# iamgroot42/A-LINK

Measured on AMD Instinct MI355X. Metric: 112x112 face embeddings/sec (IR-ResNet-100 ArcFace, 512-d, L2-normalised), higher is better.
Workload: dtype bf16

## Files before the change

a-link_amd/csrc/alink_common.h:

```cpp
#pragma once
#include <hip/hip_runtime.h>
#include <stdint.h>
#include <stddef.h>
#include <string>

#include "../../include/alink_hip.h"
#include "conv_kernel.h"

namespace alink {

void set_error(const char* fmt, ...);
int  hip_fail(hipError_t e, const char* what, const char* file, int line);

#define ALINK_HIP(call)                                                          \
    do {                                                                         \
        hipError_t e__ = (call);                                                 \
        if (e__ != hipSuccess) return ::alink::hip_fail(e__, #call, __FILE__, __LINE__); \
    } while (0)

#define ALINK_REQUIRE(cond, code, ...)          \
    do {                                        \
        if (!(cond)) {                          \
            ::alink::set_error(__VA_ARGS__);    \
            return (code);                      \
// ... 19 lines not shown
        if (dev < 0 || hipGetDevice(&prev) != hipSuccess || prev == dev) return;
        switched = hipSetDevice(dev) == hipSuccess;
    }
    ~DeviceGuard() {
        if (switched) (void)hipSetDevice(prev);
    }
    DeviceGuard(const DeviceGuard&) = delete;
    DeviceGuard& operator=(const DeviceGuard&) = delete;
};

typedef __attribute__((ext_vector_type(8))) __bf16   bf16x8;
typedef __attribute__((ext_vector_type(8))) _Float16 f16x8;
typedef __attribute__((ext_vector_type(4))) float    f32x4;
typedef __attribute__((ext_vector_type(16))) float   f32x16;

struct ConvParams {
    const void*  in;
    const void*  wgt;
    const float* bias;
    const float* alpha;
    const void*  resid;
    const void*  dact;
    void*        out;
    const void*  zero;
    const void*  in2;
    int Cin2;
    int in2_compact;
    int N, H, W, Cin, Cout, Ho, Wo, stride, ksz, pad, M;
    int border_cls;
    int splitk;
    int ksteps_per_split;
    int post_relu;
    int fine;
    int stagger;
    int ablate;
    float acc_scale;
    float bias_scale;
    float res_scale;
    int nprod;
    void* stamps;
};

hipError_t launch_conv_igemm(int dtype, const ConvParams& p, hipStream_t stream);
double     conv_flops(const ConvParams& p);

struct StemParams {
    const void*  in;
    const void*  wgt;
    const float* bias;
    const float* alpha;
    void*        out;
    int N, H, W, C0, layout;
    float sub[3], mul;
    int flip;
    float acc_scale, bias_scale;
};
hipError_t launch_stem(int dtype, const StemParams& p, hipStream_t stream);

struct FcFinishParams {
    const float* slabs;
    const float* bias;
    float*       out;
    float*       norms;
    int S, M, E;
    float scale;
    int*  nonfinite;
// ... 77 lines not shown
```

a-link_amd/csrc/backbone.hip:

```cpp
#include "alink_common.h"
#include "net_host.h"

#include <algorithm>
#include <cmath>
#include <cstdarg>
#include <cstdio>
#include <cstring>
#include <map>
#include <string>
#include <vector>

namespace alink {

static thread_local char g_err[1024] = "";
void set_error(const char* fmt, ...) {
    va_list ap;
    va_start(ap, fmt);
    vsnprintf(g_err, sizeof(g_err), fmt, ap);
    va_end(ap);
}
int hip_fail(hipError_t e, const char* what, const char* file, int line) {
    set_error("HIP error %d (%s) in `%s` at %s:%d", (int)e, hipGetErrorString(e), what, file, line);
    return ALINK_EHIP;
}
// ... 551 lines not shown
        worst = std::max(worst, sum);
    }
    return worst;
}

static int plan_split(const alink_backbone* bb, const ConvLayer& L, int N) {
    if (!bb->split_small || N > SPLIT_MAX_N || L.Cin2) return 1;
    const long long M = (long long)N * L.Hout * L.Wout;
    const int ncc = L.Cin / 64;
    const ConvKernelTraits t = traits(L.kernel);
    long long nwg;
    int units, kpu;
    if (t.split == SplitUnit::Chunk) {
        nwg = linear_grid(M, L.Cout, t.channel_block);
        units = ncc; kpu = 9;
    } else if (t.split == SplitUnit::KStep) {
        const bool wide = (L.Cout % 128) == 0;
        nwg = wide ? ((M + 127) / 128) * (L.Cout / 128) : ((M + 255) / 256) * (L.Cout / 64);
        units = L.ksz * L.ksz * ncc; kpu = 1;
    } else {
        return 1;
    }
    if (nwg > 64) return 1;
    int best = 1;
    for (int S = 2; S <= 8; ++S)
        if (units % S == 0 && units / S * kpu >= 4 && nwg * S <= 512 && (size_t)S * M * L.Cout * 4 <= SPLIT_SLAB_BYTES) best = S;
    return best;
}

int g_sibling_aware = 1;
extern "C" void alink_debug_set_sibling_aware(int on) { g_sibling_aware = on != 0; }
int g_fine_max = 384;
extern "C" void alink_debug_set_fine_max(int n) { g_fine_max = n; }
static int fine_form(ConvKernel k, long long M, int Cout, int siblings = 1) {
    if (!traits(k).fine) return 0;
    const int sib = (g_sibling_aware && k != ConvKernel::Linear7) ? siblings : 1;
    return linear_grid(M, Cout, 128) * sib <= g_fine_max ? 1 : 0;
}
int g_ablate = 0;
int g_stop_after = 0;
extern "C" void alink_debug_set_stop_after(int n) { g_stop_after = n; }
int g_stagger = 0;
int g_shard_stagger = 0;
extern "C" void alink_debug_set_shard_stagger(int on) { g_shard_stagger = on; }

int g_fuse_unit = 1;
constexpr int FUSE_UNIT_MIN_N = 64;
extern "C" void alink_debug_set_fuse_unit(int mode) { g_fuse_unit = mode; }
extern "C" void alink_debug_set_stagger(int n) { g_stagger = n < 0 ? 0 : n; }
void* g_stamps = nullptr;
int g_prof_reps = 4;
extern "C" void alink_debug_set_profile_reps(int n) { g_prof_reps = n < 1 ? 1 : n; }
extern "C" void alink_debug_set_ablate(int a) { g_ablate = a; }
extern "C" void alink_debug_set_stamps(void* p) { g_stamps = p; }

static const ConvLayer* fusable_unit(const alink_backbone* bb, const ConvLayer& L, int N, int S, bool cache) {
    if (!g_fuse_unit || (g_fuse_unit == 1 && N < FUSE_UNIT_MIN_N) || cache || S != 1 || g_ablate || g_stamps) return nullptr;
    const int dt = bb->cfg.dtype;
    if (dt != ALINK_DT_BF16 && dt != ALINK_DT_F16) return nullptr;
    const size_t i = (size_t)(&L - bb->convs.data());
    if (L.role != 1 || i + 1 >= bb->convs.size()) return nullptr;
    const ConvLayer& L2 = bb->convs[i + 1];
    if (L2.role != 3 || L2.unit != L.unit || L2.Cin2 || L2.in_buf != L.out_buf || L2.resid_buf != L.in_buf) return nullptr;
    if (L.kernel != ConvKernel::Linear56 || L2.kernel != ConvKernel::Linear56 || L.stride != 1 || L2.stride != 1) return nullptr;
    if (L.Cin != 64 || L.Cout != 64 || L2.Cin != 64 || L2.Cout != 64 || L.Hin != 56 || L.Win != 56) return nullptr;
    if (plan_split(bb, L2, N) != 1) return nullptr;
    return &L2;
}

constexpr int FUSE_UNIT1_MIN_N = 64;
// ... 63 lines not shown
        bexp[0] = bb->stem_e_out;
    } else {
        for (int r = 0; r < reps; ++r) ALINK_HIP(launch_stem(cfg.dtype, sp, stream));
    }
    if (!front) {
        note(2.0 * N * cfg.height * cfg.width * 64.0 * 27.0, 0);
        if ((rc = mark())) return rc;
    }

    int last_out = 0, n_done = 0;
    bool front_marked = false;
    bool skip_conv2 = false;
    for (ConvLayer& L : bb->convs) {
        if (skip_conv2) { skip_conv2 = false; continue; }
        if (g_stop_after && n_done++ >= g_stop_after) return ALINK_OK;
        if (front_done && !front_marked && L.stage >= 1) {
            ALINK_HIP(hipEventRecord(front_done, stream));
            front_marked = true;
        }
        ConvParams p{};
        p.in = buf(L.in_buf); p.wgt = L.d_w; p.bias = L.d_bias; p.alpha = L.d_alpha;
        p.resid = L.resid_buf >= 0 ? buf(L.resid_buf) : nullptr;
        p.out = buf(L.out_buf); p.zero = bb->d_zero;
        if (cache) {
            if (L.role == 1) p.out = base + cache->toff[L.unit];
            if (L.role == 3) p.in = base + cache->toff[L.unit];
        }
        conv_geometry(p, N, L.Hin, L.Win, L.Cin, L.Cout, L.ksz, L.stride, L.pad, L.Cin2, x2);
        p.border_cls = L.border_cls ? 1 : 0;
        if (L.Cin2) { p.in2 = buf(L.in2_buf); p.Cin2 = L.Cin2; p.in2_compact = (front && &L == &bb->convs[1]) ? 1 : 0; }
        p.ablate = g_ablate;
        p.stagger = g_stagger;
        p.nprod = (x2 && !calib) ? bb->products : 0;
        p.fine = fine_form(L.kernel, p.M, L.Cout, bb->siblings);
        int S = plan_split(bb, L, N);
        if (S > 1) {
            ConvParams probe = p;
            probe.splitk = 1;
            if (traits(L.kernel).split == SplitUnit::Chunk ? conv3x3_lat_applies(cfg.dtype, probe) : conv_gemm_lat_applies(cfg.dtype, probe)) S = 1;
        }
        if (x2) {
            rc = bb->cal.settle(calib, &L.e_out, p.out, (size_t)p.M * L.Cout * 2, stream, [&](int e) -> int {
                p.acc_scale = std::ldexp(1.f, e - bexp[L.in_buf] - L.e_w);
                p.bias_scale = std::ldexp(1.f, e);
                p.res_scale = L.resid_buf >= 0 ? std::ldexp(1.f, e - bexp[L.resid_buf]) : 1.f;
                for (int r = 0; r < reps; ++r) ALINK_HIP(launch_conv_maybe_split(L.kernel, cfg.dtype, p, S, buf(6), stream));
                return ALINK_OK;
            });
            if (rc) return rc;
            bexp[L.out_buf] = L.e_out;
        } else if (front && &L == &bb->convs[0] && fusable_unit1(bb, front, N, cache != nullptr)) {
            const ConvLayer& L2 = bb->convs[1];
            ConvParams p2 = p;
            p2.in = buf(L2.in_buf); p2.wgt = L2.d_w; p2.bias = L2.d_bias; p2.alpha = L2.d_alpha; p2.resid = nullptr;
            p2.out = buf(L2.out_buf); p2.border_cls = L2.border_cls ? 1 : 0;
            conv_geometry(p2, N, L2.Hin, L2.Win, L2.Cin, L2.Cout, L2.ksz, L2.stride, L2.pad, L2.Cin2);
            p2.in2 = buf(L2.in2_buf); p2.Cin2 = L2.Cin2; p2.in2_compact = 1;
            ALINK_REQUIRE(unit1_c64_applies(cfg.dtype, p, sp, p2), ALINK_EINVAL, "fused unit %s: launch forms do not apply", L.name.c_str());
            for (int r = 0; r < reps; ++r) ALINK_HIP(launch_unit1_c64(cfg.dtype, p, sp, p2, bb->front_slopes_le_1, stream));
            note(conv_flops(p) + 2.0 * N * cfg.height * cfg.width * 64.0 * 27.0, 1);
            if ((rc = mark())) return rc;
            if (prof && nl < cap) split_pairs.push_back(nl - 1);
            note(conv_flops(p2), 1);
            if ((rc = mark())) return rc;
            last_out = L2.out_buf;
            skip_conv2 = true;
            continue;
// ... 358 lines not shown

static int conv_nhwc_impl(int dtype, const void* dev_in, const void* dev_w, const float* dev_bias,
                          const float* dev_alpha, const void* dev_resid, void* dev_out, int N, int H, int W, int Cin,
                          int Cout, int ksz, int stride, int pad, int border_cls, int fine, const ConvExtras& x, void* stream) {
    ALINK_REQUIRE(dev_in && dev_w && dev_bias && dev_out, ALINK_EINVAL, "NULL argument");
    DeviceGuard dg(device_of_pointer(dev_in));
    ALINK_REQUIRE(Cin % 64 == 0 && Cout % 64 == 0, ALINK_EINVAL, "Cin/Cout must be multiples of 64");
    ALINK_REQUIRE(ksz == 1 || ksz == 3, ALINK_EINVAL, "ksz must be 1 or 3");
    ALINK_REQUIRE(!border_cls || (ksz == 3 && stride == 1 && pad == 1), ALINK_EINVAL,
                  "border classes need a 3x3 stride-1 pad-1 convolution");
    ALINK_REQUIRE(dtype == ALINK_DT_BF16 || dtype == ALINK_DT_F16, ALINK_EINVAL, "dtype must be bf16 or f16");
    int rc = init_kernels();
    if (rc) return rc;
    const ConvKernel kernel = x.route ? direct_variant_tiles(ksz, stride, pad, H, W, Cin, Cout)
                                      : direct_variant(ksz, stride, pad, H, W, Cin, Cout);
    if ((rc = check_extras(kernel, dtype, ksz, Cin, dev_alpha, dev_resid, x))) return rc;
    hipStream_t st = (hipStream_t)stream;
    const int K = ksz * ksz * Cin, Cin2 = x.in2 ? x.Cin2 : 0;
    std::vector<uint16_t> h((size_t)Cout * K), h2((size_t)Cout * Cin2);
    ALINK_HIP(hipStreamSynchronize(st));
    ALINK_HIP(hipMemcpy(h.data(), dev_w, h.size() * 2, hipMemcpyDeviceToHost));
    if (Cin2) ALINK_HIP(hipMemcpy(h2.data(), x.w2, h2.size() * 2, hipMemcpyDeviceToHost));
    const std::vector<uint16_t> hp =
        pack_conv_weights(weight_layout(kernel, ksz, Cin, false, Cin2), dtype, Round16::Direct, Cout,
                          [&](int co, int tap, int ci) { return (double)widen16(dtype, h[(size_t)co * K + (size_t)tap * Cin + ci]); },
                          [&](int co, int ci) { return (double)widen16(dtype, h2[(size_t)co * Cin2 + ci]); }).w;
    ConvParams p{};
    p.in = dev_in; p.bias = dev_bias; p.alpha = dev_alpha; p.resid = dev_resid; p.dact = x.dact; p.out = dev_out;
    conv_geometry(p, N, H, W, Cin, Cout, ksz, stride, pad, Cin2);
    p.border_cls = border_cls;
    p.post_relu = x.post_relu;
    if (Cin2) { p.in2 = x.in2; p.Cin2 = Cin2; p.in2_compact = x.in2_compact ? 1 : 0; }
    p.ablate = g_ablate; p.stamps = g_stamps;
    if (traits(kernel).fine) p.fine = fine < 0 ? fine_form(kernel, p.M, Cout) : (fine ? 1 : 0);
    DeviceAllocs mem;
    void *d_wp = nullptr, *d_zero = nullptr, *d_slabs = nullptr;
    if ((rc = mem.upload(hp, &d_wp)) || (rc = mem.zeros(4096, &d_zero))) return rc;
    if (x.splitk > 1 && (rc = mem.alloc((size_t)x.splitk * p.M * Cout * 4, &d_slabs))) return rc;
    p.wgt = d_wp; p.zero = d_zero;
    hipError_t e = launch_conv_reported(kernel, dtype, p, x.splitk, (float*)d_slabs, x, st);
    hipError_t e2 = hipStreamSynchronize(st);
    if (e != hipSuccess) return hip_fail(e, "launch_conv", __FILE__, __LINE__);
    if (e2 != hipSuccess) return hip_fail(e2, "hipStreamSynchronize", __FILE__, __LINE__);
    return ALINK_OK;
}

int alink_conv_nhwc(int dtype, const void* dev_in, const void* dev_w, const float* dev_bias,
                    const float* dev_alpha, const void* dev_resid, void* dev_out, int N, int H, int W, int Cin,
                    int Cout, int ksz, int stride, int pad, int border_cls, int fine, void* stream) {
    return conv_nhwc_impl(dtype, dev_in, dev_w, dev_bias, dev_alpha, dev_resid, dev_out, N, H, W, Cin, Cout, ksz, stride, pad,
                          border_cls, fine, ConvExtras{}, stream);
}

int alink_conv_nhwc_ex(int dtype, const void* dev_in, const void* dev_w, const float* dev_bias,
                       const float* dev_alpha, const void* dev_resid, void* dev_out, int N, int H, int W, int Cin,
                       int Cout, int ksz, int stride, int pad, int border_cls, int fine, int route, const void* dev_dact,
                       int post_relu, const void* dev_in2, const void* dev_w2, int Cin2, int in2_compact, int splitk,
                       int* kernel_out, int* form_out, void* stream) {
    ConvExtras x;
    x.route = route ? 1 : 0; x.dact = dev_dact; x.post_relu = post_relu ? 1 : 0;
    x.in2 = dev_in2; x.w2 = dev_w2; x.Cin2 = Cin2; x.in2_compact = in2_compact; x.splitk = splitk;
    x.kernel = kernel_out; x.form = form_out;
    if (kernel_out) *kernel_out = -1;
    if (form_out) *form_out = -1;
    return conv_nhwc_impl(dtype, dev_in, dev_w, dev_bias, dev_alpha, dev_resid, dev_out, N, H, W, Cin, Cout, ksz, stride, pad,
                          border_cls, fine, x, stream);
}
// ... 22 lines not shown
        ALINK_HIP(hipMemcpy(h.data(), dev, h.size() * 4, hipMemcpyDeviceToHost));
        q.assign(rows * C * 2, 0);
        for (size_t m = 0; m < rows; ++m)
            for (int c = 0; c < C; ++c) {
                const size_t at = m * 2 * C + (size_t)(c >> 6) * 128 + (c & 63);
                split16(std::ldexp((double)h[m * C + c], e), &q[at], &q[at + 64]);
            }
        return ALINK_OK;
    };
    std::vector<uint16_t> qin, qres, qw;
    if ((rc = pack_act(dev_in, Min, Cin, e_in, qin))) return rc;
    if (dev_resid && (rc = pack_act(dev_resid, M, Cout, e_res, qres))) return rc;
    {
        std::vector<float> h((size_t)Cout * K);
        ALINK_HIP(hipMemcpy(h.data(), dev_w, h.size() * 4, hipMemcpyDeviceToHost));
        qw = pack_conv_weights(weight_layout(kernel, ksz, Cin, true), ALINK_DT_F16X2, Round16::Direct, Cout,
                               [&](int co, int tap, int ci) { return (double)h[(size_t)co * K + (size_t)tap * Cin + ci]; },
                               [](int, int) { return 0.0; }, &e_w).w;
    }
    DeviceAllocs mem;
    void *d_in = nullptr, *d_res = nullptr, *d_w = nullptr, *d_out = nullptr, *d_zero = nullptr, *d_slabs = nullptr;
    if ((rc = mem.upload(qin, &d_in)) || (rc = mem.upload(qw, &d_w)) || (rc = mem.alloc(M * Cout * 4, &d_out)) ||
        (rc = mem.zeros(4096, &d_zero))) return rc;
    if (x.splitk > 1 && (rc = mem.alloc((size_t)x.splitk * M * Cout * 4, &d_slabs))) return rc;
    if (dev_resid && (rc = mem.upload(qres, &d_res))) return rc;
    ConvParams p{};
    p.in = d_in; p.wgt = d_w; p.bias = dev_bias; p.alpha = dev_alpha; p.resid = d_res; p.out = d_out;
    p.zero = d_zero; p.border_cls = border_cls;
    conv_geometry(p, N, H, W, Cin, Cout, ksz, stride, pad, 0, true);
    p.post_relu = x.post_relu; p.nprod = x.nprod;
    p.acc_scale = std::ldexp(1.f, e_out - e_in - e_w);
    p.bias_scale = std::ldexp(1.f, e_out);
    p.res_scale = std::ldexp(1.f, e_out - e_res);
    if (traits(kernel).fine) p.fine = fine < 0 ? fine_form(kernel, p.M, Cout) : (fine ? 1 : 0);
    ALINK_HIP(launch_conv_reported(kernel, ALINK_DT_F16X2, p, x.splitk, (float*)d_slabs, x, st));
    ALINK_HIP(hipStreamSynchronize(st));
    std::vector<uint16_t> qo(M * Cout * 2);
    ALINK_HIP(hipMemcpy(qo.data(), d_out, qo.size() * 2, hipMemcpyDeviceToHost));
    std::vector<float> ho(M * Cout);
    for (size_t m = 0; m < M; ++m)
        for (int c = 0; c < Cout; ++c) {
            const size_t at = m * 2 * Cout + (size_t)(c >> 6) * 128 + (c & 63);
            _Float16 hh, ll;
            memcpy(&hh, &qo[at], 2);
            memcpy(&ll, &qo[at + 64], 2);
            ho[m * Cout + c] = (float)std::ldexp((double)hh + (double)ll, -e_out);
        }
    ALINK_HIP(hipMemcpy(dev_out, ho.data(), ho.size() * 4, hipMemcpyHostToDevice));
    return ALINK_OK;
}

int alink_conv_nhwc_x2(const float* dev_in, const float* dev_w, const float* dev_bias, const float* dev_alpha,
                       const float* dev_resid, float* dev_out, int N, int H, int W, int Cin, int Cout, int ksz, int stride,
                       int pad, int border_cls, int fine, int e_in, int e_w, int e_out, int e_res, void* stream) {
    return conv_nhwc_x2_impl(dev_in, dev_w, dev_bias, dev_alpha, dev_resid, dev_out, N, H, W, Cin, Cout, ksz, stride, pad, border_cls,
                             fine, e_in, e_w, e_out, e_res, ConvExtras{}, stream);
}

int alink_conv_nhwc_x2_ex(const float* dev_in, const float* dev_w, const float* dev_bias, const float* dev_alpha,
                          const float* dev_resid, float* dev_out, int N, int H, int W, int Cin, int Cout, int ksz, int stride,
                          int pad, int border_cls, int fine, int e_in, int e_w, int e_out, int e_res, int nprod, int splitk,
                          int post_relu, int* kernel_out, int* form_out, void* stream) {
    ConvExtras x;
    x.nprod = nprod; x.splitk = splitk; x.post_relu = post_relu ? 1 : 0; x.kernel = kernel_out; x.form = form_out;
    if (kernel_out) *kernel_out = -1;
    if (form_out) *form_out = -1;
    return conv_nhwc_x2_impl(dev_in, dev_w, dev_bias, dev_alpha, dev_resid, dev_out, N, H, W, Cin, Cout, ksz, stride, pad, border_cls,
// ... 5 lines not shown
```

a-link_amd/csrc/conv3x3_linear.hip:

```cpp
#include "conv_device.h"

namespace alink {
namespace {

template <int A>
struct IC { static constexpr int a = A; };

constexpr int GPX = 224;
constexpr int TPW = 7;
constexpr int NT = 256;

template <int W, int TCW>
struct Lin {
    static constexpr int BN = 2 * TCW * 16;
    static constexpr int XPIX = GPX + 2 * W + 2;
    static constexpr int XSLOTS = (XPIX * 8 + NT - 1) / NT;
    static constexpr int XBYTES = XSLOTS * NT * 16;
    static constexpr int WOFF = XBYTES;
    static constexpr int WBYTES = BN * 128;
    static constexpr size_t lds_bytes() { return (size_t)WOFF + 2 * WBYTES + 10 * BN * 4; }
    static_assert(GPX % W == 0, "a workgroup covers whole rows");
};

template <typename T, int W, int TCW, int EPI, bool SP, int NP = 3>
__global__ __launch_bounds__(NT, 2) void conv3x3_linear_kernel(const ConvParams p) {
    typedef typename Vec8<T>::type vec8;
    typedef Lin<W, TCW> G;
    constexpr int BN = G::BN, XSLOTS = G::XSLOTS, WBYTES = G::WBYTES, WSLOTS = BN * 8 / NT;
    extern __shared__ __attribute__((aligned(16))) char smem[];

    const int tid = threadIdx.x, lane = tid & 63;
    const int wave = __builtin_amdgcn_readfirstlane(tid >> 6);
    const int wpx = wave >> 1, wco = wave & 1;
    if (p.stagger > 0) {
        __shared__ int s_late;
        if (tid == 0) s_late = (int)(__builtin_amdgcn_s_getreg(6148) & 1u);
        __syncthreads();
        if (s_late)
            for (int i = 0; i < p.stagger; ++i) __builtin_amdgcn_s_sleep(16);
    }
    const int q = lane >> 4, lr = lane & 15;
    const int H = p.H, Cin = p.Cin;
    unsigned long long* const stamps = (unsigned long long*)p.stamps;
    unsigned long long refill_cycles = 0;
    if (stamps && tid == 0) stamps[(size_t)blockIdx.x * 8 + 0] = __builtin_amdgcn_s_memtime();
    constexpr int NPH = SP ? NP : 1;
    const int CinP = SP ? 2 * Cin : Cin;
    const int ncc_all = Cin >> 6;
    const int ncc = ncc_all / p.splitk, cc_first = (int)blockIdx.y * ncc;
    const int nk = ncc * 9 * NPH;
    const int K = 9 * CinP;
    const long long totpix = (long long)p.N * H * W;

    const int ntn = p.Cout / BN;
    const int lid = xcd_remap(blockIdx.x, gridDim.x);
    const int tile_n = lid % ntn, grp = lid / ntn;
    const int n0 = tile_n * BN;
    const long long gp0 = (long long)grp * GPX;

    const T* __restrict__ gin = (const T*)p.in;
    const T* __restrict__ gw = (const T*)p.wgt;
    const T* __restrict__ gz = (const T*)p.zero;

    const int xpos0 = tid >> 3;
    const int xc16 = (tid & 7) ^ ((tid >> 4) & 7);
    const long long xgp0 = gp0 - W - 1 + xpos0;
    auto stage_x = [&](int cc, int part = 0) {
        long long x0 = xgp0;
        if (SP) asm volatile("" : "+v"(x0));
#pragma unroll
        for (int i = 0; i < XSLOTS; ++i) {
            const long long gp = x0 + 32 * i;
            const bool ok = xpos0 + 32 * i < G::XPIX && gp >= 0 && gp < totpix;
            const T* src = ok ? gin + ((size_t)gp * CinP + (SP ? 2 * cc + part : cc) * 64 + xc16 * 8) : gz + (lane & 7) * 8;
            dma16(src, smem + (NT * i + wave * 64) * 16);
        }
    };
    const unsigned woff0 = (unsigned)((tid >> 3) * K + (((tid & 7) ^ ((tid >> 4) & 7)) * 8));
    const T* wstep = gw + (size_t)n0 * K + (size_t)cc_first * (SP ? 18 : 9) * 64;
    int wr = 0;
    auto stage_w = [&](int bufoff) {
#pragma unroll
        for (int i = 0; i < WSLOTS; ++i)
            dma16(wstep + (woff0 + (unsigned)(32 * i * K)), smem + G::WOFF + bufoff + (NT * i + wave * 64) * 16);
        if (SP && NP == 1) {
            wstep += wr == 8 ? 10 * 64 : 64;
            wr = wr == 8 ? 0 : wr + 1;
        } else if (SP) {
            wstep += wr == 17 ? -17 * 64 : (wr == 26 ? 10 * 64 : 64);
            wr = wr == 26 ? 0 : wr + 1;
        } else {
            wstep += 64;
        }
    };

    stage_x(cc_first);
    stage_w(0);

    const int dl = delta(lr);
    const int xbase = wpx * (TPW * 2048);
    unsigned border = 0;
#pragma unroll
    for (int u = 0; u < TPW; ++u) {
        const int pl = 16 * (wpx * TPW + u) + dl;
        const int col = pl % W;
        const int y = (int)(((unsigned)grp * (unsigned)(GPX / W) + (unsigned)(pl / W)) % (unsigned)W);
        border |= ((y == 0 ? 1u : 0u) | (y == H - 1 ? 2u : 0u) | (col == 0 ? 4u : 0u) | (col == W - 1 ? 8u : 0u)) << (4 * u);
    }
    int wl[2];
    {
        const int rowb = wco * (16 * TCW) + lr;
        const int f = (lr >> 1) & 7;
        wl[0] = G::WOFF + rowb * 128 + (((0 | q) ^ f) << 4);
        wl[1] = G::WOFF + rowb * 128 + (((4 | q) ^ f) << 4);
    }

    f32x4 acc[TCW][TPW];
#pragma unroll
    for (int t = 0; t < TCW; ++t)
#pragma unroll
        for (int u = 0; u < TPW; ++u) acc[t][u] = f32x4{0.f, 0.f, 0.f, 0.f};

    const int ncls = p.border_cls ? 9 : 1;
    float* const ebias = (float*)(smem + G::WOFF + 2 * WBYTES);
    float* const ealpha = ebias + 9 * BN;
    for (int i = tid; i < ncls * BN; i += NT) ebias[i] = p.bias[(i / BN) * p.Cout + n0 + (i % BN)] * (SP ? p.bias_scale : 1.f);
    if (p.alpha)
        for (int i = tid; i < BN; i += NT) ealpha[i] = p.alpha[n0 + i];
    wait_then_barrier<0>();
    if (stamps && tid == 0) stamps[(size_t)blockIdx.x * 8 + 1] = __builtin_amdgcn_s_memtime();

    int wtog = 0;
    for (int cc = 0; cc < ncc; ++cc) {
#pragma unroll 1
      for (int ph = 0; ph < NPH; ++ph) {
        auto step = [&](auto tapc) {
            constexpr int tap = decltype(tapc)::a;
            constexpr int ky = tap / 3, kx = tap % 3;
            constexpr unsigned tapbits = (ky == 0 ? 1u : 0u) | (ky == 2 ? 2u : 0u) | (kx == 0 ? 4u : 0u) | (kx == 2 ? 8u : 0u);
            const int t = (cc * NPH + ph) * 9 + tap;
            if (t + 1 < nk) stage_w(wtog ^ WBYTES);
            unsigned bnow = border;
            int sdl = dl;
            asm volatile("" : "+v"(bnow), "+v"(sdl));
            const int spos = sdl + ky * W + kx;
            const int xt0 = xbase + spos * 128 + ((q ^ ((spos >> 1) & 7)) << 4);
            const int xt1 = xt0 ^ 64;
#pragma unroll
            for (int ks = 0; ks < 2; ++ks) {
                vec8 wf[TCW], pf[TPW];
#pragma unroll
                for (int tt = 0; tt < TCW; ++tt) wf[tt] = *(const vec8*)(smem + (wl[ks] + wtog) + tt * 2048);
#pragma unroll
                for (int u = 0; u < TPW; ++u) {
                    const unsigned t = tapbits ? (bnow & (tapbits << (4 * u))) : 0u;
                    const unsigned far = 4 * u < 18 ? t << (18 - (4 * u < 18 ? 4 * u : 0)) : t;
                    pf[u] = *(const vec8*)(smem + ((ks ? xt1 : xt0) + (int)far) + 2048 * u);
                }
#pragma unroll
                for (int tt = 0; tt < TCW; ++tt)
#pragma unroll
// ... 76 lines not shown
                vec8 res[TPW][CPL / 8];
#pragma unroll
                for (int u = 0; u < TPW; ++u)
#pragma unroll
                    for (int h = 0; h < CPL / 8; ++h) res[u][h] = *(const vec8*)(r + off[u] + so[h] + 64 * part);
#pragma unroll
                for (int u = 0; u < TPW; ++u)
#pragma unroll
                    for (int h = 0; h < CPL / 8; ++h)
#pragma unroll
                        for (int i = 0; i < 8; ++i)
                            acc[2 * h + (i >> 2)][u][i & 3] = fmaf((float)res[u][h][i], p.res_scale, acc[2 * h + (i >> 2)][u][i & 3]);
            }
        }
#pragma unroll
        for (int u = 0; u < TPW; ++u) {
            if (!ok[u]) continue;
#pragma unroll
            for (int h = 0; h < CPL / 8; ++h) {
                vec8 o8, l8;
#pragma unroll
                for (int i = 0; i < 8; ++i) {
                    float v = acc[2 * h + (i >> 2)][u][i & 3];
                    if (EPI == 0 && p.post_relu) v = relu_keep_nan(v);
                    o8[i] = (T)v;
                    l8[i] = (T)(v - (float)o8[i]);
                }
                *(vec8*)((T*)p.out + off[u] + so[h]) = o8;
                *(vec8*)((T*)p.out + off[u] + so[h] + 64) = l8;
            }
        }
        return;
    }
    size_t off[TPW];
    bool ok[TPW];
    int cls[TPW];
#pragma unroll
    for (int u = 0; u < TPW; ++u) {
        const long long gp = gp0 + 16 * (wpx * TPW + u) + dl;
        ok[u] = gp < totpix;
        off[u] = (size_t)(ok[u] ? gp : 0) * p.Cout + n0;
        const unsigned b4 = (border >> (4 * u)) & 15u;
        const int rc = (b4 & 1u) ? 0 : ((b4 & 2u) ? 2 : 1);
        const int ccl = (b4 & 4u) ? 0 : ((b4 & 8u) ? 2 : 1);
        cls[u] = p.border_cls ? rc * 3 + ccl : 0;
    }
    vec8 res[TPW][CPL / 8];
    const T* extra = EPI == 1 ? (const T*)nullptr : (const T*)((EPI == 0 && p.dact) ? p.dact : p.resid);
    if (EPI == 2 || (EPI == 0 && extra)) {
#pragma unroll
        for (int u = 0; u < TPW; ++u)
#pragma unroll
            for (int h = 0; h < CPL / 8; ++h) res[u][h] = *(const vec8*)(extra + off[u] + chan_h(h));
    }
    if (stamps) {
        asm volatile("s_waitcnt vmcnt(0)" ::: "memory");
        if (tid == 0) stamps[(size_t)blockIdx.x * 8 + 6] = __builtin_amdgcn_s_memtime();
    }
#pragma unroll
    for (int u = 0; u < TPW; ++u) {
        float v[CPL];
#pragma unroll
        for (int t = 0; t < TCW; ++t) {
            const f32x4 b4 = *(const f32x4*)(ebias + cls[u] * BN + chan_t(t));
#pragma unroll
            for (int j = 0; j < 4; ++j) v[4 * t + j] = acc[t][u][j] + b4[j];
        }
        if (EPI == 0 && p.dact) {
#pragma unroll
            for (int t = 0; t < TCW; ++t) {
                const f32x4 a4 = *(const f32x4*)(ealpha + chan_t(t));
#pragma unroll
                for (int j = 0; j < 4; ++j) v[4 * t + j] *= (float)res[u][(4 * t + j) / 8][(4 * t + j) % 8] > 0.f ? 1.f : a4[j];
            }
        } else {
            if (EPI == 1 || (EPI == 0 && p.alpha)) {
#pragma unroll
                for (int t = 0; t < TCW; ++t) {
                    const f32x4 a4 = *(const f32x4*)(ealpha + chan_t(t));
#pragma unroll
                    for (int j = 0; j < 4; ++j) v[4 * t + j] = v[4 * t + j] > 0.f ? v[4 * t + j] : v[4 * t + j] * a4[j];
                }
            }
            if (EPI == 2 || (EPI == 0 && p.resid)) {
#pragma unroll
                for (int h = 0; h < CPL / 8; ++h)
#pragma unroll
                    for (int i = 0; i < 8; ++i) v[8 * h + i] += (float)res[u][h][i];
            }
        }
        if (EPI == 0 && p.post_relu) {
#pragma unroll
            for (int i = 0; i < CPL; ++i) v[i] = relu_keep_nan(v[i]);
        }
        if (ok[u]) {
#pragma unroll
            for (int h = 0; h < CPL / 8; ++h) {
                vec8 o8;
#pragma unroll
                for (int i = 0; i < 8; ++i) o8[i] = (T)v[8 * h + i];
                *(vec8*)((T*)p.out + off[u] + chan_h(h)) = o8;
            }
        }
    }
    if (stamps && tid == 0) {
        stamps[(size_t)blockIdx.x * 8 + 7] = __builtin_amdgcn_s_memtime();
        asm volatile("s_waitcnt vmcnt(0)" ::: "memory");
        stamps[(size_t)blockIdx.x * 8 + 3] = __builtin_amdgcn_s_memtime();
    }
}

bool g_generic_epilogue = false;

template <typename T, int W, int TCW, bool SP = false>
hipError_t launch_one(const ConvParams& p, hipStream_t st) {
    typedef Lin<W, TCW> G;
    const long long totpix = (long long)p.N * p.H * W;
    const long long groups = (totpix + GPX - 1) / GPX;
    const long long nwg = groups * (p.Cout / G::BN);
    if (nwg <= 0 || nwg >= (1ll << 31)) return hipErrorInvalidValue;
    const dim3 grid((unsigned)nwg, (unsigned)p.splitk);
    if (SP) {
        if (p.dact) return hipErrorInvalidValue;
        if (p.nprod == 1) {
            if (p.splitk > 1) hipLaunchKernelGGL((conv3x3_linear_kernel<T, W, TCW, 3, SP, 1>), grid, dim3(NT), G::lds_bytes(), st, p);
            else              hipLaunchKernelGGL((conv3x3_linear_kernel<T, W, TCW, 0, SP, 1>), grid, dim3(NT), G::lds_bytes(), st, p);
            return hipGetLastError();
        }
        const bool plain_sp = p.splitk == 1 && !p.post_relu && !p.stamps && !g_generic_epilogue;
        if (p.splitk > 1) hipLaunchKernelGGL((conv3x3_linear_kernel<T, W, TCW, 3, SP>), grid, dim3(NT), G::lds_bytes(), st, p);
        else if (plain_sp && p.alpha && !p.resid)
            hipLaunchKernelGGL((conv3x3_linear_kernel<T, W, TCW, 1, SP>), grid, dim3(NT), G::lds_bytes(), st, p);
        else if (plain_sp && !p.alpha && p.resid)
            hipLaunchKernelGGL((conv3x3_linear_kernel<T, W, TCW, 2, SP>), grid, dim3(NT), G::lds_bytes(), st, p);
        else              hipLaunchKernelGGL((conv3x3_linear_kernel<T, W, TCW, 0, SP>), grid, dim3(NT), G::lds_bytes(), st, p);
        return hipGetLastError();
    }
// ... 72 lines not shown
bool g_contract_ok[64] = {};
}
hipError_t linear_check_contract() {
    const int dev = current_device();
    float* d = nullptr;
    hipError_t e = hipMalloc((void**)&d, PROBE_FLOATS * sizeof(float));
    if (e != hipSuccess) return e;
    float h[PROBE_FLOATS];
    for (int i = 0; i < PROBE_FLOATS; ++i) h[i] = 7.f;
    e = hipMemcpy(d, h, sizeof(h), hipMemcpyHostToDevice);
    if (e == hipSuccess) {
        hipLaunchKernelGGL(lds_oob_probe_kernel, dim3(1), dim3(64), 0, (hipStream_t)0, d);
        e = hipGetLastError();
    }
    if (e == hipSuccess) e = hipMemcpy(h, d, sizeof(h), hipMemcpyDeviceToHost);
    (void)hipFree(d);
    if (e != hipSuccess) return e;
    bool ok = h[512] == 1.f && h[513] == 2.f && h[514] == 3.f && h[515] == 4.f;
    for (int i = 0; i < 512; ++i) ok = ok && h[i] == 0.f;
    if (dev >= 0 && dev < 64) g_contract_ok[dev] = ok;
    return hipSuccess;
}

extern "C" int alink_debug_lds_oob_probe(float* dev_out516, void* stream) {
    DeviceGuard dg(device_of_pointer(dev_out516));
    hipLaunchKernelGGL(lds_oob_probe_kernel, dim3(1), dim3(64), 0, (hipStream_t)stream, dev_out516);
    return hipGetLastError() == hipSuccess ? 0 : -1;
}
extern "C" int alink_debug_linear_contract_ok(void) {
    const int dev = current_device();
    return dev >= 0 && dev < 64 && g_contract_ok[dev] ? 1 : 0;
}

ConvKernel linear_variant(int ksz, int stride, int pad, int H, int W, int Cin, int Cout) {
    if (ksz != 3 || stride != 1 || pad != 1 || H != W || Cin % 64) return ConvKernel::Igemm;
    const int dev = current_device();
    if (dev < 0 || dev >= 64 || !g_contract_ok[dev]) return ConvKernel::Igemm;
    if ((g_linear_mode & 4) && W == 14 && Cout % 128 == 0) return ConvKernel::Linear14;
    if ((g_linear_mode & 2) && W == 28 && Cout % 128 == 0) return ConvKernel::Linear28;
    if ((g_linear_mode & 1) && W == 56 && Cout % 64 == 0) return ConvKernel::Linear56;
    if ((g_linear_mode & 8) && W == 7 && Cout % 128 == 0) return ConvKernel::Linear7;
    return ConvKernel::Igemm;
}
ConvKernel linear_variant_x2(int ksz, int stride, int pad, int H, int W, int Cin, int Cout) {
    const ConvKernel k = linear_variant(ksz, stride, pad, H, W, Cin, Cout);
    if (k != ConvKernel::Igemm) return k;
    if (ksz != 3 || stride != 1 || pad != 1 || H != W || Cin % 64) return ConvKernel::Igemm;
    const int dev = current_device();
    if (dev < 0 || dev >= 64 || !g_contract_ok[dev]) return ConvKernel::Igemm;
    if ((g_linear_mode & 16) && W == 112 && Cout % 64 == 0) return ConvKernel::Linear112;
    return ConvKernel::Igemm;
}

hipError_t linear_set_attributes() {
    hipError_t e;
#define A(T)                                                              \
    if ((e = set_attr_one<T, 14, 4>()) != hipSuccess) return e;           \
    if ((e = set_attr_one<T, 28, 4>()) != hipSuccess) return e;           \
    if ((e = set_attr_one<T, 56, 2>()) != hipSuccess) return e;           \
    if ((e = set_attr_one<T, 7, 4>()) != hipSuccess) return e;            \
    if ((e = set_attr_one<T, 14, 2>()) != hipSuccess) return e;           \
    if ((e = set_attr_one<T, 28, 2>()) != hipSuccess) return e;           \
    if ((e = set_attr_one<T, 7, 2>()) != hipSuccess) return e;
    A(__bf16) A(_Float16)
#undef A
#define B(W_, TCW_) if ((e = set_attr_sp<W_, TCW_>()) != hipSuccess) return e;
    B(14, 4) B(28, 4) B(56, 2) B(7, 4) B(14, 2) B(28, 2) B(7, 2) B(112, 2)
#undef B
    return hipSuccess;
}

hipError_t launch_conv3x3_linear(ConvKernel k, int dtype, const ConvParams& p, hipStream_t st) {
    if (p.ksz != 3 || p.stride != 1 || p.pad != 1 || p.H != p.W) return hipErrorInvalidValue;
    if (conv3x3_lat_applies(dtype, p)) return launch_conv3x3_lat(dtype, p, st);
    if (p.splitk < 1 || (p.Cin / 64) % p.splitk) return hipErrorInvalidValue;
    if ((long long)p.N * p.H * p.W * p.Cin * (dtype == ALINK_DT_F16X2 ? 2 : 1) >= (1ll << 31)) return hipErrorInvalidValue;
#define L(W_, TCW_) (dtype == ALINK_DT_BF16 ? launch_one<__bf16, W_, TCW_>(p, st) : (dtype == ALINK_DT_F16X2 ? launch_one<_Float16, W_, TCW_, true>(p, st) : launch_one<_Float16, W_, TCW_>(p, st)))
    if (p.fine) {
        switch (k) {
            case ConvKernel::Linear14: return p.W == 14 ? L(14, 2) : hipErrorInvalidValue;
            case ConvKernel::Linear28: return p.W == 28 ? L(28, 2) : hipErrorInvalidValue;
            case ConvKernel::Linear7:  return p.W == 7 ? L(7, 2) : hipErrorInvalidValue;
            default: break;
        }
    }
    switch (k) {
        case ConvKernel::Linear14:  return p.W == 14 ? L(14, 4) : hipErrorInvalidValue;
        case ConvKernel::Linear28:  return p.W == 28 ? L(28, 4) : hipErrorInvalidValue;
        case ConvKernel::Linear56:  return p.W == 56 ? L(56, 2) : hipErrorInvalidValue;
        case ConvKernel::Linear7:   return p.W == 7 ? L(7, 4) : hipErrorInvalidValue;
        case ConvKernel::Linear112: return p.W == 112 && dtype == ALINK_DT_F16X2 ? launch_one<_Float16, 112, 2, true>(p, st) : hipErrorInvalidValue;
        default: break;
    }
#undef L
    return hipErrorInvalidValue;
}

}
```

a-link_amd/csrc/conv_kernel.h:

```cpp
#pragma once
#include <stddef.h>

namespace alink {

enum class ConvKernel : int {
    Igemm = 0,
    TileW14C256 = 1,
    TileW28C256 = 2,
    TileW28C128 = 3,
    TileW56C128 = 4,
    TileW56C64 = 5,
    TileW112C64 = 6,
    PairW14C128 = 7,
    PairW28C128 = 8,
    Linear14 = 11,
    Linear28 = 12,
    Linear56 = 13,
    Linear7 = 14,
    Linear112 = 15,
    Roll112 = 21,
    Roll112S2 = 25,
};

enum class SplitUnit { None, Chunk, KStep };

struct ConvKernelTraits {
    int       row_perm;
    bool      chunk_major;
    int       channel_block;
    bool      fine;
    SplitUnit split;
};

inline ConvKernelTraits traits(ConvKernel k) {
    switch (k) {
        case ConvKernel::Igemm:       return {16, false, 0, false, SplitUnit::KStep};
        case ConvKernel::TileW14C256:
        case ConvKernel::TileW28C256:
        case ConvKernel::PairW14C128:
        case ConvKernel::PairW28C128: return {17, true, 0, false, SplitUnit::None};
        case ConvKernel::TileW28C128:
        case ConvKernel::TileW56C128:
        case ConvKernel::TileW56C64:
        case ConvKernel::TileW112C64: return {8, true, 0, false, SplitUnit::None};
        case ConvKernel::Linear14:
        case ConvKernel::Linear28:
        case ConvKernel::Linear7:     return {17, true, 128, true, SplitUnit::Chunk};
        case ConvKernel::Linear56:
        case ConvKernel::Linear112:   return {8, true, 64, false, SplitUnit::Chunk};
        case ConvKernel::Roll112:
        case ConvKernel::Roll112S2:   return {8, true, 0, false, SplitUnit::None};
    }
    return {16, false, 0, false, SplitUnit::None};
}

inline long long linear_grid(long long M, int Cout, int channel_block) { return (M + 223) / 224 * (Cout / channel_block); }

static inline int perm64_row_of_channel(int c) {
    int q = c >> 4, t = (c >> 2) & 3, j = c & 3;
    return 16 * t + 4 * q + j;
}
static inline int perm32_row_of_channel(int c) {
    int q = c >> 3, t = (c >> 2) & 1, j = c & 3;
    return 16 * t + 4 * q + j;
}
static inline int perm64b_row_of_channel(int c) {
    int th = c >> 5, q = (c >> 3) & 3, tl = (c >> 2) & 1, j = c & 3;
    return 16 * (2 * th + tl) + 4 * q + j;
}
static inline int permuted_row(int co, int cpl) {
    if (cpl == 17) return (co & ~63) + perm64b_row_of_channel(co & 63);
    return cpl == 16 ? (co & ~63) + perm64_row_of_channel(co & 63) : (co & ~31) + perm32_row_of_channel(co & 31);
}

struct WeightLayout {
    int  row_perm;
    bool chunk_major, split;
    int  taps, cin, cin2;

    size_t row_pitch() const { return split ? (size_t)2 * taps * cin : (size_t)taps * cin + cin2; }
    size_t size(int rows) const { return (size_t)rows * row_pitch(); }
// ... 16 lines not shown
```

include/alink_hip_debug.h:

```cpp
#ifndef ALINK_HIP_DEBUG_H
#define ALINK_HIP_DEBUG_H

#include <stddef.h>

#ifdef __cplusplus
extern "C" {
#endif

void alink_debug_set_linear(int mode);
void alink_debug_set_generic_epilogue(int on);
void alink_debug_set_direct(int on);
void alink_debug_set_pair(int on);
void alink_debug_set_c64(int on);
void alink_debug_set_s2direct(int on);
void alink_debug_set_fuse_stem(int on);
void alink_debug_set_fuse_unit(int mode);
void alink_debug_set_fuse_unit1(int mode);
void alink_debug_set_fuse_shortcut(int on);
void alink_debug_set_dma(int on);
void alink_debug_set_fine_max(int n);
void alink_debug_set_sibling_aware(int on);
void alink_debug_set_latency_form(int max_pixels);
void alink_debug_set_latency_tiles(int form);
void alink_debug_set_stagger(int n);
void alink_debug_set_shard_stagger(int on);

void alink_debug_set_tiny_step(int on);
void alink_debug_set_mini_step(int on);
void alink_debug_set_head_bf16_mfma(int on);

void alink_debug_set_smallres_overlap(int on);
void alink_debug_set_smallres_one_update(int on);

void alink_debug_set_stop_after(int n);
void alink_debug_set_profile_reps(int n);
void alink_debug_set_ablate(int a);
void alink_debug_set_stamps(void* dev_u64);
int alink_debug_lds_oob_probe(float* dev_out516, void* stream);
int alink_debug_linear_contract_ok(void);


struct alink_resnet50;
struct alink_backbone;
int alink_debug_resnet50_grad_cache_info(const struct alink_resnet50* r, int n_images, int index, size_t* byte_offset, int* H,
                                         int* W, int* C, char* name_buf, int name_len);
int alink_debug_backbone_grad_cache_info(const struct alink_backbone* bb, int n_images, int index, size_t* byte_offset, int* H,
                                         int* W, int* C, char* name_buf, int name_len);

#ifdef __cplusplus
}
#endif
#endif
```

Measured before the change: 46900.

## Add wide 4-tile form for the 56x56 linear 3x3 conv kernel

Enables a wider output-channel tile (TCW=4, covering 128 channels) for the Linear56 3x3 conv, chosen by default when Cout is a multiple of 128 and dtype is not f16x2. This lets each input tile staged in LDS be reused across more output channels. It also shrinks the activation staging buffer to its exact pixel count by handling the final partial slot with a shifted tail DMA, which saves LDS. The cost is higher LDS and register pressure per block, which may lower occupancy; a debug occupancy query and a mode switch are added to check and control this.

```diff
diff --git a/a-link_amd/csrc/alink_common.h b/a-link_amd/csrc/alink_common.h
--- a/a-link_amd/csrc/alink_common.h
+++ b/a-link_amd/csrc/alink_common.h
@@ -75,6 +75,7 @@
     int ksteps_per_split;
     int post_relu;
     int fine;
+    int wide;
     int stagger;
     int ablate;
     float acc_scale;
diff --git a/a-link_amd/csrc/backbone.hip b/a-link_amd/csrc/backbone.hip
--- a/a-link_amd/csrc/backbone.hip
+++ b/a-link_amd/csrc/backbone.hip
@@ -607,10 +607,21 @@
 extern "C" void alink_debug_set_sibling_aware(int on) { g_sibling_aware = on != 0; }
 int g_fine_max = 384;
 extern "C" void alink_debug_set_fine_max(int n) { g_fine_max = n; }
-static int fine_form(ConvKernel k, long long M, int Cout, int siblings = 1) {
+int g_linear56_wide = 1;
+extern "C" void alink_debug_set_linear56_wide(int mode) { g_linear56_wide = mode; }
+static int fine_form(ConvKernel k, int dtype, long long M, int Cout, int siblings = 1) {
     if (!traits(k).fine) return 0;
+    if (k == ConvKernel::Linear56) {
+        if (Cout % 128 || dtype == ALINK_DT_F16X2 || g_linear56_wide == 0) return 1;
+        if (g_linear56_wide == 2) return 0;
+    }
     const int sib = (g_sibling_aware && k != ConvKernel::Linear7) ? siblings : 1;
     return linear_grid(M, Cout, 128) * sib <= g_fine_max ? 1 : 0;
+}
+static void set_form(ConvParams& p, ConvKernel k, int fine) {
+    if (!traits(k).fine) return;
+    if (traits(k).channel_block == 128) p.fine = fine;
+    else p.wide = fine ? 0 : 1;
 }
 int g_ablate = 0;
 int g_stop_after = 0;
@@ -740,7 +751,7 @@
         p.ablate = g_ablate;
         p.stagger = g_stagger;
         p.nprod = (x2 && !calib) ? bb->products : 0;
-        p.fine = fine_form(L.kernel, p.M, L.Cout, bb->siblings);
+        set_form(p, L.kernel, fine_form(L.kernel, cfg.dtype, p.M, L.Cout, bb->siblings));
         int S = plan_split(bb, L, N);
         if (S > 1) {
             ConvParams probe = p;
@@ -1165,7 +1176,7 @@
     p.post_relu = x.post_relu;
     if (Cin2) { p.in2 = x.in2; p.Cin2 = Cin2; p.in2_compact = x.in2_compact ? 1 : 0; }
     p.ablate = g_ablate; p.stamps = g_stamps;
-    if (traits(kernel).fine) p.fine = fine < 0 ? fine_form(kernel, p.M, Cout) : (fine ? 1 : 0);
+    set_form(p, kernel, fine < 0 ? fine_form(kernel, dtype, p.M, Cout) : ((fine || (kernel == ConvKernel::Linear56 && Cout % 128)) ? 1 : 0));
     DeviceAllocs mem;
     void *d_wp = nullptr, *d_zero = nullptr, *d_slabs = nullptr;
     if ((rc = mem.upload(hp, &d_wp)) || (rc = mem.zeros(4096, &d_zero))) return rc;
@@ -1254,7 +1265,7 @@
     p.acc_scale = std::ldexp(1.f, e_out - e_in - e_w);
     p.bias_scale = std::ldexp(1.f, e_out);
     p.res_scale = std::ldexp(1.f, e_out - e_res);
-    if (traits(kernel).fine) p.fine = fine < 0 ? fine_form(kernel, p.M, Cout) : (fine ? 1 : 0);
+    if (kernel != ConvKernel::Linear56) set_form(p, kernel, fine < 0 ? fine_form(kernel, ALINK_DT_F16X2, p.M, Cout) : (fine ? 1 : 0));
     ALINK_HIP(launch_conv_reported(kernel, ALINK_DT_F16X2, p, x.splitk, (float*)d_slabs, x, st));
     ALINK_HIP(hipStreamSynchronize(st));
     std::vector<uint16_t> qo(M * Cout * 2);
diff --git a/a-link_amd/csrc/conv3x3_linear.hip b/a-link_amd/csrc/conv3x3_linear.hip
--- a/a-link_amd/csrc/conv3x3_linear.hip
+++ b/a-link_amd/csrc/conv3x3_linear.hip
@@ -1,4 +1,8 @@
 #include "conv_device.h"
+
+#ifndef ALINK_LINEAR_REBUILD_X
+#define ALINK_LINEAR_REBUILD_X 0
+#endif
 
 namespace alink {
 namespace {
@@ -15,7 +19,10 @@
     static constexpr int BN = 2 * TCW * 16;
     static constexpr int XPIX = GPX + 2 * W + 2;
     static constexpr int XSLOTS = (XPIX * 8 + NT - 1) / NT;
-    static constexpr int XBYTES = XSLOTS * NT * 16;
+    static constexpr int XBYTES = XPIX * 128;
+    static constexpr int XTAIL = XPIX - 32 * (XSLOTS - 1);
+    static constexpr int XTAILW = XTAIL / 8;
+    static constexpr int XTAILR = XTAIL % 8;
     static constexpr int WOFF = XBYTES;
     static constexpr int WBYTES = BN * 128;
     static constexpr size_t lds_bytes() { return (size_t)WOFF + 2 * WBYTES + 10 * BN * 4; }
@@ -67,13 +74,20 @@
     const long long xgp0 = gp0 - W - 1 + xpos0;
     auto stage_x = [&](int cc, int part = 0) {
         long long x0 = xgp0;
-        if (SP) asm volatile("" : "+v"(x0));
+        if (SP || (W == 56 && TCW == 4) || ALINK_LINEAR_REBUILD_X) asm volatile("" : "+v"(x0));
+        const int coff = (SP ? 2 * cc + part : cc) * 64;
 #pragma unroll
         for (int i = 0; i < XSLOTS; ++i) {
-            const long long gp = x0 + 32 * i;
-            const bool ok = xpos0 + 32 * i < G::XPIX && gp >= 0 && gp < totpix;
-            const T* src = ok ? gin + ((size_t)gp * CinP + (SP ? 2 * cc + part : cc) * 64 + xc16 * 8) : gz + (lane & 7) * 8;
-            dma16(src, smem + (NT * i + wave * 64) * 16);
+            int back = 0;
+            if (i == XSLOTS - 1) {
+                if (wave > G::XTAILW || (wave == G::XTAILW && !G::XTAILR)) continue;
+                if (wave == G::XTAILW) back = 8 - G::XTAILR;
+            }
+            const long long gp = x0 + 32 * i - back;
+            const int c16 = back ? (tid & 7) ^ (((xpos0 - back) >> 1) & 7) : xc16;
+            const bool ok = gp >= 0 && gp < totpix;
+            const T* src = ok ? gin + ((size_t)gp * CinP + coff + c16 * 8) : gz + (lane & 7) * 8;
+            dma16(src, smem + (NT * i + wave * 64 - back * 8) * 16);
         }
     };
     const unsigned woff0 = (unsigned)((tid >> 3) * K + (((tid & 7) ^ ((tid >> 4) & 7)) * 8));
@@ -478,6 +492,20 @@
     return dev >= 0 && dev < 64 && g_contract_ok[dev] ? 1 : 0;
 }
 
+extern "C" int alink_debug_linear56_wide_occupancy(int dtype, int epi, int* lds_bytes) {
+    if (init_kernels()) return -1;
+    const size_t lds = Lin<56, 4>::lds_bytes();
+    if (lds_bytes) *lds_bytes = (int)lds;
+    const void* f = nullptr;
+#define K(T, E) (const void*)conv3x3_linear_kernel<T, 56, 4, E, false>
+    if (dtype == ALINK_DT_BF16)     f = epi == 0 ? K(__bf16, 0) : (epi == 1 ? K(__bf16, 1) : (epi == 2 ? K(__bf16, 2) : nullptr));
+    else if (dtype == ALINK_DT_F16) f = epi == 0 ? K(_Float16, 0) : (epi == 1 ? K(_Float16, 1) : (epi == 2 ? K(_Float16, 2) : nullptr));
+#undef K
+    int n = -1;
+    if (!f || hipOccupancyMaxActiveBlocksPerMultiprocessor(&n, f, NT, lds) != hipSuccess) return -1;
+    return n;
+}
+
 ConvKernel linear_variant(int ksz, int stride, int pad, int H, int W, int Cin, int Cout) {
     if (ksz != 3 || stride != 1 || pad != 1 || H != W || Cin % 64) return ConvKernel::Igemm;
     const int dev = current_device();
@@ -504,6 +532,7 @@
     if ((e = set_attr_one<T, 14, 4>()) != hipSuccess) return e;           \
     if ((e = set_attr_one<T, 28, 4>()) != hipSuccess) return e;           \
     if ((e = set_attr_one<T, 56, 2>()) != hipSuccess) return e;           \
+    if ((e = set_attr_one<T, 56, 4>()) != hipSuccess) return e;           \
     if ((e = set_attr_one<T, 7, 4>()) != hipSuccess) return e;            \
     if ((e = set_attr_one<T, 14, 2>()) != hipSuccess) return e;           \
     if ((e = set_attr_one<T, 28, 2>()) != hipSuccess) return e;           \
@@ -522,6 +551,7 @@
     if (p.splitk < 1 || (p.Cin / 64) % p.splitk) return hipErrorInvalidValue;
     if ((long long)p.N * p.H * p.W * p.Cin * (dtype == ALINK_DT_F16X2 ? 2 : 1) >= (1ll << 31)) return hipErrorInvalidValue;
 #define L(W_, TCW_) (dtype == ALINK_DT_BF16 ? launch_one<__bf16, W_, TCW_>(p, st) : (dtype == ALINK_DT_F16X2 ? launch_one<_Float16, W_, TCW_, true>(p, st) : launch_one<_Float16, W_, TCW_>(p, st)))
+#define L16(W_, TCW_) (dtype == ALINK_DT_BF16 ? launch_one<__bf16, W_, TCW_>(p, st) : launch_one<_Float16, W_, TCW_>(p, st))
     if (p.fine) {
         switch (k) {
             case ConvKernel::Linear14: return p.W == 14 ? L(14, 2) : hipErrorInvalidValue;
@@ -533,12 +563,16 @@
     switch (k) {
         case ConvKernel::Linear14:  return p.W == 14 ? L(14, 4) : hipErrorInvalidValue;
         case ConvKernel::Linear28:  return p.W == 28 ? L(28, 4) : hipErrorInvalidValue;
-        case ConvKernel::Linear56:  return p.W == 56 ? L(56, 2) : hipErrorInvalidValue;
+        case ConvKernel::Linear56:
+            if (p.W != 56) return hipErrorInvalidValue;
+            if (p.wide) return p.Cout % 128 == 0 && dtype != ALINK_DT_F16X2 ? L16(56, 4) : hipErrorInvalidValue;
+            return L(56, 2);
         case ConvKernel::Linear7:   return p.W == 7 ? L(7, 4) : hipErrorInvalidValue;
         case ConvKernel::Linear112: return p.W == 112 && dtype == ALINK_DT_F16X2 ? launch_one<_Float16, 112, 2, true>(p, st) : hipErrorInvalidValue;
         default: break;
     }
 #undef L
+#undef L16
     return hipErrorInvalidValue;
 }
 
diff --git a/a-link_amd/csrc/conv_kernel.h b/a-link_amd/csrc/conv_kernel.h
--- a/a-link_amd/csrc/conv_kernel.h
+++ b/a-link_amd/csrc/conv_kernel.h
@@ -46,7 +46,7 @@
         case ConvKernel::Linear14:
         case ConvKernel::Linear28:
         case ConvKernel::Linear7:     return {17, true, 128, true, SplitUnit::Chunk};
-        case ConvKernel::Linear56:
+        case ConvKernel::Linear56:    return {8, true, 64, true, SplitUnit::Chunk};
         case ConvKernel::Linear112:   return {8, true, 64, false, SplitUnit::Chunk};
         case ConvKernel::Roll112:
         case ConvKernel::Roll112S2:   return {8, true, 0, false, SplitUnit::None};
diff --git a/include/alink_hip_debug.h b/include/alink_hip_debug.h
--- a/include/alink_hip_debug.h
+++ b/include/alink_hip_debug.h
@@ -19,6 +19,8 @@
 void alink_debug_set_fuse_shortcut(int on);
 void alink_debug_set_dma(int on);
 void alink_debug_set_fine_max(int n);
+void alink_debug_set_linear56_wide(int mode);
+int alink_debug_linear56_wide_occupancy(int dtype, int epi, int* lds_bytes);
 void alink_debug_set_sibling_aware(int on);
 void alink_debug_set_latency_form(int max_pixels);
 void alink_debug_set_latency_tiles(int form);
```

New measurement: 47150 (median of 6 runs). Within noise of the previous version (+0.5%).

## Prefetch bias/alpha tables early, split full-tile epilogue, drop stamps in fused epilogues

Applied to the files above, without the earlier changes.

The bias and PReLU slope loads are issued into registers right after the first DMA stage, so their global latency overlaps the input staging, and they are written to LDS later. The epilogue becomes a lambda instantiated twice: a full-tile version with no bounds checks and a tail version, plus a sched_barrier after the residual loads. Timing stamps are compiled out for EPI 1/2. This adds register pressure from the held table values and duplicates code, which may affect occupancy or I-cache.

```diff
diff --git a/a-link_amd/csrc/conv3x3_linear.hip b/a-link_amd/csrc/conv3x3_linear.hip
--- a/a-link_amd/csrc/conv3x3_linear.hip
+++ b/a-link_amd/csrc/conv3x3_linear.hip
@@ -41,7 +41,7 @@
     }
     const int q = lane >> 4, lr = lane & 15;
     const int H = p.H, Cin = p.Cin;
-    unsigned long long* const stamps = (unsigned long long*)p.stamps;
+    unsigned long long* const stamps = (EPI == 1 || EPI == 2) ? nullptr : (unsigned long long*)p.stamps;
     unsigned long long refill_cycles = 0;
     if (stamps && tid == 0) stamps[(size_t)blockIdx.x * 8 + 0] = __builtin_amdgcn_s_memtime();
     constexpr int NPH = SP ? NP : 1;
@@ -96,6 +96,19 @@
 
     stage_x(cc_first);
     stage_w(0);
+    const int ncls = p.border_cls ? 9 : 1;
+    constexpr int TBL_TRIPS = (9 * BN + NT - 1) / NT;
+    static_assert(BN <= NT, "the slope table is one trip");
+    float tbias[TBL_TRIPS], talpha;
+#pragma unroll
+    for (int k = 0; k < TBL_TRIPS; ++k) {
+        const int i = tid + NT * k;
+        tbias[k] = p.bias[i < ncls * BN ? (i / BN) * p.Cout + n0 + (i % BN) : 0];
+    }
+    {
+        const float* ap = p.alpha ? p.alpha + n0 + (tid < BN ? tid : 0) : p.bias;
+        talpha = *ap;
+    }
 
     const int dl = delta(lr);
     const int xbase = wpx * (TPW * 2048);
@@ -121,12 +134,20 @@
 #pragma unroll
         for (int u = 0; u < TPW; ++u) acc[t][u] = f32x4{0.f, 0.f, 0.f, 0.f};
 
-    const int ncls = p.border_cls ? 9 : 1;
+    asm volatile("" : "+v"(border));
+#pragma unroll
+    for (int t = 0; t < TCW; ++t)
+#pragma unroll
+        for (int u = 0; u < TPW; ++u) asm volatile("" : "+v"(acc[t][u]));
+
     float* const ebias = (float*)(smem + G::WOFF + 2 * WBYTES);
     float* const ealpha = ebias + 9 * BN;
-    for (int i = tid; i < ncls * BN; i += NT) ebias[i] = p.bias[(i / BN) * p.Cout + n0 + (i % BN)] * (SP ? p.bias_scale : 1.f);
-    if (p.alpha)
-        for (int i = tid; i < BN; i += NT) ealpha[i] = p.alpha[n0 + i];
+#pragma unroll
+    for (int k = 0; k < TBL_TRIPS; ++k) {
+        const int i = tid + NT * k;
+        if (i < ncls * BN) ebias[i] = tbias[k] * (SP ? p.bias_scale : 1.f);
+    }
+    if (p.alpha && tid < BN) ealpha[tid] = talpha;
     wait_then_barrier<0>();
     if (stamps && tid == 0) stamps[(size_t)blockIdx.x * 8 + 1] = __builtin_amdgcn_s_memtime();
 
@@ -269,77 +290,83 @@
         }
         return;
     }
-    size_t off[TPW];
-    bool ok[TPW];
-    int cls[TPW];
-#pragma unroll
-    for (int u = 0; u < TPW; ++u) {
-        const long long gp = gp0 + 16 * (wpx * TPW + u) + dl;
-        ok[u] = gp < totpix;
-        off[u] = (size_t)(ok[u] ? gp : 0) * p.Cout + n0;
-        const unsigned b4 = (border >> (4 * u)) & 15u;
-        const int rc = (b4 & 1u) ? 0 : ((b4 & 2u) ? 2 : 1);
-        const int ccl = (b4 & 4u) ? 0 : ((b4 & 8u) ? 2 : 1);
-        cls[u] = p.border_cls ? rc * 3 + ccl : 0;
-    }
-    vec8 res[TPW][CPL / 8];
-    const T* extra = EPI == 1 ? (const T*)nullptr : (const T*)((EPI == 0 && p.dact) ? p.dact : p.resid);
-    if (EPI == 2 || (EPI == 0 && extra)) {
-#pragma unroll
-        for (int u = 0; u < TPW; ++u)
-#pragma unroll
-            for (int h = 0; h < CPL / 8; ++h) res[u][h] = *(const vec8*)(extra + off[u] + chan_h(h));
-    }
-    if (stamps) {
-        asm volatile("s_waitcnt vmcnt(0)" ::: "memory");
-        if (tid == 0) stamps[(size_t)blockIdx.x * 8 + 6] = __builtin_amdgcn_s_memtime();
-    }
-#pragma unroll
-    for (int u = 0; u < TPW; ++u) {
-        float v[CPL];
-#pragma unroll
-        for (int t = 0; t < TCW; ++t) {
-            const f32x4 b4 = *(const f32x4*)(ebias + cls[u] * BN + chan_t(t));
-#pragma unroll
-            for (int j = 0; j < 4; ++j) v[4 * t + j] = acc[t][u][j] + b4[j];
-        }
-        if (EPI == 0 && p.dact) {
+    auto epilogue16 = [&](auto fullc) {
+        constexpr bool FULL = decltype(fullc)::a != 0;
+        size_t off[TPW];
+        bool ok[TPW];
+        int cls[TPW];
+#pragma unroll
+        for (int u = 0; u < TPW; ++u) {
+            const long long gp = gp0 + 16 * (wpx * TPW + u) + dl;
+            ok[u] = FULL || gp < totpix;
+            off[u] = (size_t)(FULL || ok[u] ? gp : 0) * p.Cout + n0;
+            const unsigned b4 = (border >> (4 * u)) & 15u;
+            const int rc = (b4 & 1u) ? 0 : ((b4 & 2u) ? 2 : 1);
+            const int ccl = (b4 & 4u) ? 0 : ((b4 & 8u) ? 2 : 1);
+            cls[u] = p.border_cls ? rc * 3 + ccl : 0;
+        }
+        vec8 res[TPW][CPL / 8];
+        const T* extra = EPI == 1 ? (const T*)nullptr : (const T*)((EPI == 0 && p.dact) ? p.dact : p.resid);
+        if (EPI == 2 || (EPI == 0 && extra)) {
+#pragma unroll
+            for (int u = 0; u < TPW; ++u)
+#pragma unroll
+                for (int h = 0; h < CPL / 8; ++h) res[u][h] = *(const vec8*)(extra + off[u] + chan_h(h));
+            __builtin_amdgcn_sched_barrier(0);
+        }
+        if (stamps) {
+            asm volatile("s_waitcnt vmcnt(0)" ::: "memory");
+            if (tid == 0) stamps[(size_t)blockIdx.x * 8 + 6] = __builtin_amdgcn_s_memtime();
+        }
+#pragma unroll
+        for (int u = 0; u < TPW; ++u) {
+            float v[CPL];
 #pragma unroll
             for (int t = 0; t < TCW; ++t) {
-                const f32x4 a4 = *(const f32x4*)(ealpha + chan_t(t));
-#pragma unroll
-                for (int j = 0; j < 4; ++j) v[4 * t + j] *= (float)res[u][(4 * t + j) / 8][(4 * t + j) % 8] > 0.f ? 1.f : a4[j];
-            }
-        } else {
-            if (EPI == 1 || (EPI == 0 && p.alpha)) {
+                const f32x4 b4 = *(const f32x4*)(ebias + cls[u] * BN + chan_t(t));
+#pragma unroll
+                for (int j = 0; j < 4; ++j) v[4 * t + j] = acc[t][u][j] + b4[j];
+            }
+            if (EPI == 0 && p.dact) {
 #pragma unroll
                 for (int t = 0; t < TCW; ++t) {
                     const f32x4 a4 = *(const f32x4*)(ealpha + chan_t(t));
 #pragma unroll
-                    for (int j = 0; j < 4; ++j) v[4 * t + j] = v[4 * t + j] > 0.f ? v[4 * t + j] : v[4 * t + j] * a4[j];
+                    for (int j = 0; j < 4; ++j) v[4 * t + j] *= (float)res[u][(4 * t + j) / 8][(4 * t + j) % 8] > 0.f ? 1.f : a4[j];
                 }
-            }
-            if (EPI == 2 || (EPI == 0 && p.resid)) {
-#pragma unroll
-                for (int h = 0; h < CPL / 8; ++h)
-#pragma unroll
-                    for (int i = 0; i < 8; ++i) v[8 * h + i] += (float)res[u][h][i];
-            }
-        }
-        if (EPI == 0 && p.post_relu) {
-#pragma unroll
-            for (int i = 0; i < CPL; ++i) v[i] = relu_keep_nan(v[i]);
-        }
-        if (ok[u]) {
-#pragma unroll
-            for (int h = 0; h < CPL / 8; ++h) {
-                vec8 o8;
-#pragma unroll
-                for (int i = 0; i < 8; ++i) o8[i] = (T)v[8 * h + i];
-                *(vec8*)((T*)p.out + off[u] + chan_h(h)) = o8;
-            }
-        }
-    }
+            } else {
+                if (EPI == 1 || (EPI == 0 && p.alpha)) {
+#pragma unroll
+                    for (int t = 0; t < TCW; ++t) {
+                        const f32x4 a4 = *(const f32x4*)(ealpha + chan_t(t));
+#pragma unroll
+                        for (int j = 0; j < 4; ++j) v[4 * t + j] = v[4 * t + j] > 0.f ? v[4 * t + j] : v[4 * t + j] * a4[j];
+                    }
+                }
+                if (EPI == 2 || (EPI == 0 && p.resid)) {
+#pragma unroll
+                    for (int h = 0; h < CPL / 8; ++h)
+#pragma unroll
+                        for (int i = 0; i < 8; ++i) v[8 * h + i] += (float)res[u][h][i];
+                }
+            }
+            if (EPI == 0 && p.post_relu) {
+#pragma unroll
+                for (int i = 0; i < CPL; ++i) v[i] = relu_keep_nan(v[i]);
+            }
+            if (FULL || ok[u]) {
+#pragma unroll
+                for (int h = 0; h < CPL / 8; ++h) {
+                    vec8 o8;
+#pragma unroll
+                    for (int i = 0; i < 8; ++i) o8[i] = (T)v[8 * h + i];
+                    *(vec8*)((T*)p.out + off[u] + chan_h(h)) = o8;
+                }
+            }
+        }
+    };
+    if (gp0 + GPX <= totpix) epilogue16(IC<1>{});
+    else                     epilogue16(IC<0>{});
     if (stamps && tid == 0) {
         stamps[(size_t)blockIdx.x * 8 + 7] = __builtin_amdgcn_s_memtime();
         asm volatile("s_waitcnt vmcnt(0)" ::: "memory");
```

Measured after the change: 47930 before, 48980 after, median of 6. 1.02x the previous value.
